# KyungMinJin/OTPose

Hardware: AMD Instinct MI355X
Metric: frames/sec at 384x288, 5-frame window, batch 16; heatmap max-abs delta vs ref (higher is better)
Workload: dtype f32 storage+accumulate / f16x3 split products; 1 GPU; BASELINE configs[1]: batch 16 x 5-frame x 384x288, HRNet-W48 + DCN warp + ConvVideoTransformer, fp32 forward (eval), seeded synthetic weights; clips_per_gpu=16, parallelism=dp1, outputs_finite=True

## Files before the change

### otpose_amd/csrc/convs.hip

```cpp
#include "x3.h"
#include <cstdlib>

namespace {

#ifdef OTP_CONVS_TIMING
__device__ unsigned long long otp_convs_stamps[8192 * 32];
#define SSTAMP(slot)                                                                                  \
    do {                                                                                              \
        if (threadIdx.x == 0 && blockIdx.x < 8192) otp_convs_stamps[blockIdx.x * 32 + (slot)] = __builtin_readcyclecounter(); \
    } while (0)
#else
#define SSTAMP(slot)
#endif

struct SPlan {
    int N, C, H, W, HW, Cout, total;
    int out_ctot, out_coff, act, f32_mode, res_s8;
    float pre, post;
    int NTW, nN, nTiles, nChunks, tpx;
    int NPT;
    int VR, W1, NIW, NV, pl;
    uint32_t mHW, mW, mW1, mVR;
    unsigned* rflag;
};

__global__ __launch_bounds__(256) void s8_pack_kernel(const float* __restrict__ in, otp_u32x4* __restrict__ out, float* __restrict__ c4,
                                                       int N, int C, int HW, int ctot, int coff, unsigned* rflag) {
    const int G8 = C >> 3;
    const size_t items = (size_t)N * G8 * HW;
    bool bad = false;
    for (size_t i = (size_t)blockIdx.x * 256 + threadIdx.x; i < items; i += (size_t)gridDim.x * 256) {
        const int p = (int)(i % HW);
        const size_t r = i / HW;
        const int g = (int)(r % G8), n = (int)(r / G8);
        const float* src = in + ((size_t)n * ctot + coff + 8 * g) * HW + p;
        float f[8];
#pragma unroll
        for (int e = 0; e < 8; ++e) f[e] = src[(size_t)e * HW];
#pragma unroll
        for (int e = 0; e < 8; ++e) bad |= otp_out_of_range(f[e]);
        otp_u32x4 hi, lo;
        otp_x3_split8(f, hi, lo);
        otp_u32x4* dst = out + ((size_t)(n * G8 + g) * 2) * HW + p;
        dst[0] = hi;
        dst[HW] = lo;
        if (c4) {
            otp_f32x4* d4 = reinterpret_cast<otp_f32x4*>(c4) + ((size_t)n * (C >> 2) + 2 * g) * HW + p;
            d4[0] = (otp_f32x4){f[0], f[1], f[2], f[3]};
            d4[HW] = (otp_f32x4){f[4], f[5], f[6], f[7]};
        }
    }
    otp_range_report(rflag, bad, OTP_RANGE_S8PASS);
}

struct S8Up {
    const float* low[3];
    int f[3];
    int n;
};
__global__ __launch_bounds__(256) void s8_upsample_add4_kernel(S8Up U, const float* __restrict__ res, float* out_nchw,
                                                               otp_u32x4* __restrict__ out_s8, float* __restrict__ out_c4, int N, int C,
                                                               int Hh, int Wh, int relu, int res_ctot, int res_coff, int out_ctot,
                                                               int out_coff, int res_s8, unsigned* rflag) {
    const int HW = Hh * Wh, q4 = HW >> 2, G8 = C >> 3, Wh4 = Wh >> 2;
    const size_t items = (size_t)N * G8 * q4;
    bool bad = false;
    for (size_t i = (size_t)blockIdx.x * 256 + threadIdx.x; i < items; i += (size_t)gridDim.x * 256) {
        const int q = (int)(i % q4);
        const size_t r = i / q4;
        const int g = (int)(r % G8), n = (int)(r / G8);
        const int y = q / Wh4, x4 = q - y * Wh4;
        otp_f32x4 v[8];
        if (res_s8) {
            const otp_u32x4* rs = reinterpret_cast<const otp_u32x4*>(res) + ((size_t)(n * G8 + g) * 2) * HW + 4 * q;
#pragma unroll
            for (int k = 0; k < 4; ++k) {
                const otp_u32x4 h = rs[k], l = rs[(size_t)HW + k];
#pragma unroll
                for (int e2 = 0; e2 < 4; ++e2) {
                    const otp_f32x2 a = otp_x3_widen(h[e2]) + otp_x3_widen(l[e2]);
                    v[2 * e2][k] = a.x;
                    v[2 * e2 + 1][k] = a.y;
                }
            }
        }
#pragma unroll
        for (int e = 0; e < 8; ++e) {
            const int c = 8 * g + e;
            otp_f32x4 o = res_s8 ? v[e] : *reinterpret_cast<const otp_f32x4*>(res + ((size_t)n * res_ctot + res_coff + c) * HW + 4 * q);
#pragma unroll
            for (int k = 0; k < 3; ++k) {
                if (k < U.n) {
                    const int f = U.f[k], Wl = Wh / f, Hl = Hh / f;
                    const float* lrow = U.low[k] + (((size_t)n * C + c) * Hl + y / f) * Wl;
                    if (f >= 4) {
                        o = o + lrow[(4 * x4) / f];
                    } else {
                        const float l0 = lrow[2 * x4], l1 = lrow[2 * x4 + 1];
                        o = o + (otp_f32x4){l0, l0, l1, l1};
                    }
                }
            }
#pragma unroll
            for (int j = 0; j < 4; ++j) bad |= otp_out_of_range(o[j]);
            if (relu) {
#pragma unroll
                for (int j = 0; j < 4; ++j) o[j] = fmaxf(o[j], 0.f);
            }
            v[e] = o;
            if (out_nchw) *reinterpret_cast<otp_f32x4*>(out_nchw + ((size_t)n * out_ctot + out_coff + c) * HW + 4 * q) = o;
        }
        otp_u32x4* dst = out_s8 + ((size_t)(n * G8 + g) * 2) * HW + 4 * q;
#pragma unroll
        for (int k = 0; k < 4; ++k) {
            float f[8];
#pragma unroll
            for (int e = 0; e < 8; ++e) f[e] = v[e][k];
            otp_u32x4 hi, lo;
            otp_x3_split8(f, hi, lo);
            dst[k] = hi;
            dst[(size_t)HW + k] = lo;
            if (out_c4) {
                otp_f32x4* d4 = reinterpret_cast<otp_f32x4*>(out_c4) + ((size_t)n * (C >> 2) + 2 * g) * HW + 4 * q + k;
                d4[0] = (otp_f32x4){f[0], f[1], f[2], f[3]};
                d4[HW] = (otp_f32x4){f[4], f[5], f[6], f[7]};
            }
        }
    }
    otp_range_report(rflag, bad, OTP_RANGE_S8PASS);
}

__global__ __launch_bounds__(256) void s8_upsample_add_kernel(S8Up U, const float* __restrict__ res, float* out_nchw,
                                                               otp_u32x4* __restrict__ out_s8, float* __restrict__ out_c4, int N, int C,
                                                               int Hh, int Wh, int relu, int res_ctot, int res_coff, int out_ctot,
                                                               int out_coff, int res_s8, unsigned* rflag) {
    const int HW = Hh * Wh, G8 = C >> 3;
    const size_t items = (size_t)N * G8 * HW;
    bool bad = false;
    for (size_t i = (size_t)blockIdx.x * 256 + threadIdx.x; i < items; i += (size_t)gridDim.x * 256) {
        const int p = (int)(i % HW);
        const size_t r = i / HW;
        const int g = (int)(r % G8), n = (int)(r / G8);
        const int y = p / Wh, x = p - y * Wh;
        int lo_off[3];
#pragma unroll
        for (int k = 0; k < 3; ++k) {
            const int f = k < U.n ? U.f[k] : 1;
            lo_off[k] = (y / f) * (Wh / f) + x / f;
        }
        float f8[8];
        if (res_s8) {
            const otp_u32x4* rs = reinterpret_cast<const otp_u32x4*>(res) + ((size_t)(n * G8 + g) * 2) * HW + p;
            const otp_u32x4 h = rs[0], l = rs[HW];
#pragma unroll
            for (int e2 = 0; e2 < 4; ++e2) {
                const otp_f32x2 a = otp_x3_widen(h[e2]) + otp_x3_widen(l[e2]);
                f8[2 * e2] = a.x;
                f8[2 * e2 + 1] = a.y;
            }
        }
#pragma unroll
        for (int e = 0; e < 8; ++e) {
            const int c = 8 * g + e;
            float o = res_s8 ? f8[e] : res[((size_t)n * res_ctot + res_coff + c) * HW + p];
#pragma unroll
            for (int k = 0; k < 3; ++k) {
                if (k < U.n) {
                    const int f = U.f[k];
                    o = o + U.low[k][((size_t)n * C + c) * (size_t)((Hh / f) * (Wh / f)) + lo_off[k]];
                }
            }
            bad |= otp_out_of_range(o);
            if (relu) o = fmaxf(o, 0.f);
            f8[e] = o;
            if (out_nchw) out_nchw[((size_t)n * out_ctot + out_coff + c) * HW + p] = o;
        }
        otp_u32x4 hi, lo;
        otp_x3_split8(f8, hi, lo);
        otp_u32x4* dst = out_s8 + ((size_t)(n * G8 + g) * 2) * HW + p;
        dst[0] = hi;
        dst[HW] = lo;
        if (out_c4) {
            otp_f32x4* d4 = reinterpret_cast<otp_f32x4*>(out_c4) + ((size_t)n * (C >> 2) + 2 * g) * HW + p;
            d4[0] = (otp_f32x4){f8[0], f8[1], f8[2], f8[3]};
            d4[HW] = (otp_f32x4){f8[4], f8[5], f8[6], f8[7]};
        }
    }
    otp_range_report(rflag, bad, OTP_RANGE_S8PASS);
}

__global__ __launch_bounds__(256) void c4_unpack_kernel(const otp_f32x4* __restrict__ in, float* __restrict__ out, int N, int C, int HW) {
    const size_t items = (size_t)N * (C >> 2) * HW;
    for (size_t i = (size_t)blockIdx.x * 256 + threadIdx.x; i < items; i += (size_t)gridDim.x * 256) {
        const int p = (int)(i % HW);
        const size_t r = i / HW;
        const int c4 = (int)(r % (C >> 2)), n = (int)(r / (C >> 2));
        const otp_f32x4 v = in[i];
#pragma unroll
        for (int e = 0; e < 4; ++e) out[((size_t)n * C + 4 * c4 + e) * HW + p] = v[e];
    }
}

__global__ __launch_bounds__(256) void s8_unpack_kernel(const otp_u32x4* __restrict__ in, float* __restrict__ out, int N, int C, int HW) {
    const int G8 = C >> 3;
    const size_t items = (size_t)N * G8 * HW;
    for (size_t i = (size_t)blockIdx.x * 256 + threadIdx.x; i < items; i += (size_t)gridDim.x * 256) {
        const int p = (int)(i % HW);
        const size_t r = i / HW;
        const int g = (int)(r % G8), n = (int)(r / G8);
        const otp_u32x4 hi = in[((size_t)(n * G8 + g) * 2) * HW + p], lo = in[((size_t)(n * G8 + g) * 2 + 1) * HW + p];
#pragma unroll
        for (int e = 0; e < 8; ++e) {
            const otp_f32x2 fh = otp_x3_widen(hi[e >> 1]), fl = otp_x3_widen(lo[e >> 1]);
            out[((size_t)n * C + 8 * g + e) * HW + p] = fh[e & 1] + fl[e & 1];
        }
    }
}

__global__ void s8_wpack_kernel(const float* __restrict__ w, const float* __restrict__ scale, otp_u32x4* __restrict__ out, int Cout,
                                int Cin, int NTW, int nN, int nChunks) {
    const int total = nN * nChunks * OTP_S8_KS * NTW * 64;
    const int WU = otp_s8_wch(NTW) * 64;
    for (int idx = blockIdx.x * blockDim.x + threadIdx.x; idx < total; idx += gridDim.x * blockDim.x) {
        const int lane = idx & 63;
        int r = idx >> 6;
        const int t = r % NTW; r /= NTW;
        const int s = r % OTP_S8_KS; r /= OTP_S8_KS;
        const int chunk = r % nChunks, cb = r / nChunks;
        const int cout = otp_row2ch(cb * NTW * 16, t, lane & 15, NTW, Cout), kl = lane >> 4;
        const int q = 4 * s + kl, tap = q >> 1, ci0 = chunk * 16 + 8 * (q & 1);
        if (tap > 8) continue;
        float v[8];
#pragma unroll
        for (int j = 0; j < 8; ++j) {
            const int ci = ci0 + j;
            v[j] = (cout < Cout && ci < Cin) ? w[((size_t)cout * Cin + ci) * 9 + tap] * (scale ? scale[cout] : 1.f) : 0.f;
        }
        otp_u32x4 hi, lo;
        otp_x3_split8(v, hi, lo);
        const size_t base = (size_t)(cb * nChunks + chunk) * WU;
        if (s < OTP_S8_KS - 1) {
            const size_t o = base + ((s * NTW + t) * 2) * 64 + lane;
            out[o] = hi;
            out[o + 64] = lo;
        } else {
            const size_t o = base + (OTP_S8_KS - 1) * NTW * 128 + t * 64 + lane;
            out[o] = hi;
            out[o + 32] = lo;
        }
    }
}


template <int NM>
__device__ __forceinline__ void sblock_sched_n(int nr) {
    if (nr == 0) otp_s8_block_sched<NM, 0>();
    else if (nr == 1) otp_s8_block_sched<NM, 1>();
    else if (nr == 2) otp_s8_block_sched<NM, 2>();
    else if (nr == 1 + 2 * 2) otp_s8_block_sched<NM, 1 + 2 * 2>();
    else if (nr == 2 + 2 * 2) otp_s8_block_sched<NM, 2 + 2 * 2>();
    else if (nr == 1 + 2 * 3) otp_s8_block_sched<NM, 1 + 2 * 3>();
    else otp_s8_block_sched<NM, 2 + 2 * 3>();
}

enum { S_F32_NONE = 0, S_F32_C4 = 1, S_F32_NCHW = 2 };

template <int NTW, bool NCHW, int NPT>
__global__ __launch_bounds__(256, NCHW ? 2 : 3) void convs_kernel(const unsigned char* __restrict__ xs, const otp_u32x4* __restrict__ wpk,
                                                        const float* __restrict__ shift, const float* res, float* outf,
                                                        otp_u32x4* outs, const SPlan P) {
    constexpr int BM = 64 * NPT;
    constexpr int WCH = otp_s8_wch(NTW);
    constexpr int WBYTES = WCH * 1024;
    constexpr int NBLK = OTP_S8_KS * NPT;
    constexpr int NM = 3 * NTW;
    extern __shared__ __attribute__((aligned(16))) unsigned char smem[];
    const int PL = P.pl;
    unsigned char* win = smem;
    unsigned char* wl = smem + 4 * PL;
    const int tid = threadIdx.x, lane = tid & 63;
    const int wave = __builtin_amdgcn_readfirstlane(tid >> 6);
    const int i16 = lane & 15, kl = lane >> 4;
    const bool upper = kl >= 2;

    const int xcd = (int)blockIdx.x & 7, jb = (int)blockIdx.x >> 3;
    const int tl = jb / P.nN, cb = jb - tl * P.nN;
    const int tile = xcd * P.tpx + tl;
    if (tile >= P.nTiles) return;
    SSTAMP(0);
#ifdef OTP_CONVS_TIMING
    if (threadIdx.x == 0 && blockIdx.x < 8192) otp_convs_stamps[blockIdx.x * 32 + 30] = __builtin_amdgcn_s_memrealtime();
#endif
    const int P0 = tile * BM;
    const int n0 = P0 / P.HW, p0 = P0 - n0 * P.HW;
    const int y0 = (int)otp_magic_div((uint32_t)p0, P.mW);
    const int x0 = p0 - y0 * P.W;
    const int Vf = n0 * P.VR + y0;
    const int imgB = P.C * P.HW * 4;
    const int co_blk = cb * NTW * 16;
    const int C4o = P.Cout >> 2;

    int voff[2];
    bool vlive[2];
#pragma unroll
    for (int j = 0; j < 2; ++j) {
        vlive[j] = 64 * (wave + 4 * j) + lane < P.NV;
        const int v = 64 * (wave + 4 * j) + lane + x0;
        const int r = (int)otp_magic_div((uint32_t)v, P.mW1), cp = v - otp_mul24(r, P.W1);
        const int V = Vf + r;
        const int n = (int)otp_magic_div((uint32_t)V, P.mVR), yy = V - otp_mul24(n, P.VR);
        const bool ok = cp >= 1 && yy >= 1 && n < P.N;
        voff[j] = ok ? (n - n0) * imgB + (otp_mul24(yy - 1, P.W) + cp - 1) * 16 : OTP_OOB;
    }
    const size_t left = (size_t)(P.N - n0) * imgB;
    const otp_rsrc rin = make_rsrc32(xs + (size_t)n0 * imgB, left > 0x7fffff00ull ? 0x7fffff00u : (unsigned)left);
    const otp_rsrc rw = make_rsrc32(wpk, (unsigned)((size_t)P.nN * P.nChunks * WBYTES));
    const int woff = lane * 16;

    auto stage = [&](int c) __attribute__((always_inline)) {
#pragma unroll
        for (int pl = 0; pl < 4; ++pl) {
            const int so = (((2 * c + (pl >> 1)) * 2 + (pl & 1)) * P.HW) * 16;
#pragma unroll
            for (int j = 0; j < 2; ++j) {
                const int k = wave + 4 * j;
                if (k < P.NIW && vlive[j])
                    __builtin_amdgcn_raw_ptr_buffer_load_lds(rin, (__attribute__((address_space(3))) void*)(win + pl * PL + k * 1024),
                                                             16, voff[j], so, 0, 0);
            }
        }
        const int wb = (cb * P.nChunks + c) * WBYTES;
#pragma unroll
        for (int j = 0; j < (WCH + 3) / 4; ++j) {
            const int k = wave + 4 * j;
            if (k < WCH)
                __builtin_amdgcn_raw_ptr_buffer_load_lds(rw, (__attribute__((address_space(3))) void*)(wl + k * 1024), 16, woff,
                                                         wb + k * 1024, 0, 0);
        }
    };
    stage(0);
    SSTAMP(1);

    const size_t obytes = (size_t)P.N * P.Cout * P.HW * 4;
    const otp_rsrc rres = make_rsrc32(res ? res : reinterpret_cast<const float*>(xs), res ? (unsigned)obytes : 0u);
    const otp_rsrc rs8 = make_rsrc32(outs, outs ? (unsigned)obytes : 0u);
    const otp_rsrc rof = make_rsrc32(outf, !outf ? 0u : (P.f32_mode == S_F32_C4 ? (unsigned)obytes
                                                                               : (unsigned)((size_t)P.N * P.out_ctot * P.HW * 4)));
    const otp_rsrc rsh = make_rsrc32(shift ? shift : reinterpret_cast<const float*>(xs), shift ? (unsigned)(P.Cout * 4) : 0u);
    int pb[NPT], toff[OTP_S8_KS], offN[NCHW ? NPT : 1], offS[NPT], ch0[NTW];
    otp_f32x4 acc[NTW][NPT];
    {
#pragma unroll
        for (int s = 0; s < OTP_S8_KS; ++s) {
            const int q = 4 * s + kl;
            int tap = q >> 1;
            if (tap > 8) tap = 8;
            const int dy = tap / 3, dx = tap - dy * 3;
            toff[s] = (dy * P.W1 + dx - x0) * 16 + (q & 1) * (2 * PL);
        }
        if (upper) toff[OTP_S8_KS - 1] += PL;
        otp_f32x4 sh[NTW];
#pragma unroll
        for (int t = 0; t < NTW; ++t) {
            ch0[t] = otp_row2ch(co_blk, t, 4 * kl, NTW, P.Cout);
            sh[t] = __builtin_bit_cast(otp_f32x4, __builtin_amdgcn_raw_buffer_load_b128(rsh, co_blk + 16 * t < P.Cout ? ch0[t] * 4 : OTP_OOB, 0, 0));
        }
#pragma unroll
        for (int p = 0; p < NPT; ++p) {
            int m = (wave * NPT + p) * 16 + i16;
            const bool pv = P0 + m < P.total;
            if (!pv) m = P.total - 1 - P0;
            const int q = p0 + m;
            const int dn = (int)otp_magic_div((uint32_t)q, P.mHW), pi = q - otp_mul24(dn, P.HW);
            const int y = (int)otp_magic_div((uint32_t)pi, P.mW), x = pi - otp_mul24(y, P.W);
            pb[p] = (otp_mul24(otp_mul24(n0 + dn, P.VR) + y - Vf, P.W1) + x) * 16;
            const int img = n0 + dn;
            const int c4o = (otp_mul24(otp_mul24(img, C4o), P.HW) + pi) * 16;
            if (NCHW) offN[NCHW ? p : 0] = pv ? (otp_mul24(otp_mul24(img, P.out_ctot) + P.out_coff, P.HW) + pi) * 4 : OTP_OOB;
            offS[p] = pv ? c4o : OTP_OOB;
            if (!P.res_s8) {
#pragma unroll
                for (int t = 0; t < NTW; ++t) {
                    const bool tv = co_blk + 16 * t < P.Cout;
                    acc[t][p] = __builtin_bit_cast(otp_f32x4, __builtin_amdgcn_raw_buffer_load_b128(
                        rres, (pv && tv) ? c4o + otp_mul24(ch0[t] >> 2, P.HW) * 16 : OTP_OOB, 0, 0));
                }
            }
        }
        if (P.res_s8) {
#pragma unroll
            for (int t = 1; t < NTW; t += 2)
#pragma unroll
                for (int p = 0; p < NPT; ++p) acc[t][p] = otp_f32x4{0.f, 0.f, 0.f, 0.f};
#pragma unroll
            for (int t = 0; t < NTW; t += 2) {
                const bool tav = co_blk + 16 * t < P.Cout;
                const int so = otp_mul24(ch0[t] >> 3, P.HW) * 32;
                if (otp_tile_paired(co_blk, t, NTW, P.Cout)) {
#pragma unroll
                    for (int p = 0; p < NPT; ++p) {
                        const int o = (tav && offS[p] != OTP_OOB) ? offS[p] + so : OTP_OOB;
                        const otp_u32x4 h = __builtin_bit_cast(otp_u32x4, __builtin_amdgcn_raw_buffer_load_b128(rres, o, 0, 0));
                        const otp_u32x4 l = __builtin_bit_cast(otp_u32x4, __builtin_amdgcn_raw_buffer_load_b128(rres, o, P.HW * 16, 0));
                        const otp_f32x2 a0 = otp_x3_widen(h[0]) + otp_x3_widen(l[0]), a1 = otp_x3_widen(h[1]) + otp_x3_widen(l[1]);
                        const otp_f32x2 a2 = otp_x3_widen(h[2]) + otp_x3_widen(l[2]), a3 = otp_x3_widen(h[3]) + otp_x3_widen(l[3]);
                        acc[t][p] = otp_f32x4{a0.x, a0.y, a1.x, a1.y};
                        acc[t + 1 < NTW ? t + 1 : t][p] = otp_f32x4{a2.x, a2.y, a3.x, a3.y};
                    }
                } else {
                    const int half = (ch0[t] >> 2) & 1;
#pragma unroll
                    for (int p = 0; p < NPT; ++p) {
                        const int o = (tav && offS[p] != OTP_OOB) ? offS[p] + so + 8 * half : OTP_OOB;
                        const otp_u32x2 h = __builtin_bit_cast(otp_u32x2, __builtin_amdgcn_raw_buffer_load_b64(rres, o, 0, 0));
                        const otp_u32x2 l = __builtin_bit_cast(otp_u32x2, __builtin_amdgcn_raw_buffer_load_b64(rres, o, P.HW * 16, 0));
                        const otp_f32x2 a0 = otp_x3_widen(h[0]) + otp_x3_widen(l[0]), a1 = otp_x3_widen(h[1]) + otp_x3_widen(l[1]);
                        acc[t][p] = otp_f32x4{a0.x, a0.y, a1.x, a1.y};
                    }
                }
            }
        }
#pragma unroll
        for (int t = 0; t < NTW; ++t) {
            const otp_f32x4 shp = sh[t] * P.pre;
#pragma unroll
            for (int p = 0; p < NPT; ++p) acc[t][p] = acc[t][p] * P.pre + shp;
        }
    }

    auto mfma_phase = [&]() __attribute__((always_inline)) {
        otp_x3x8 ah[2][NTW], al[2][NTW], bh[3], bl[3];
        auto load_a = [&](int buf, int s) __attribute__((always_inline)) {
#pragma unroll
            for (int t = 0; t < NTW; ++t) {
                if (s < OTP_S8_KS - 1) {
                    const unsigned char* a = wl + ((s * NTW + t) * 2) * 1024 + lane * 16;
                    ah[buf][t] = *reinterpret_cast<const otp_x3x8*>(a);
                    al[buf][t] = *reinterpret_cast<const otp_x3x8*>(a + 1024);
                } else {
                    const unsigned char* a = wl + (OTP_S8_KS - 1) * NTW * 2048 + t * 1024;
                    const otp_x3x8 h = *reinterpret_cast<const otp_x3x8*>(a + (lane & 31) * 16);
                    const otp_x3x8 z = __builtin_bit_cast(otp_x3x8, (otp_u32x4){0u, 0u, 0u, 0u});
                    al[buf][t] = *reinterpret_cast<const otp_x3x8*>(a + (lane ^ 32) * 16);
                    ah[buf][t] = upper ? z : h;
                }
            }
        };
        auto load_b = [&](int buf, int blk) __attribute__((always_inline)) {
            const unsigned char* b = win + (pb[blk % NPT] + toff[blk / NPT]);
            bh[buf] = *reinterpret_cast<const otp_x3x8*>(b);
            if (blk / NPT < OTP_S8_KS - 1) bl[buf] = *reinterpret_cast<const otp_x3x8*>(b + PL);
        };
        load_a(0, 0);
        load_b(0, 0);
        load_b(1, 1);
#pragma unroll
        for (int blk = 0; blk < NBLK; ++blk) {
            const int s = blk / NPT, p = blk % NPT, cur = blk % 3, sa = s & 1;
            const bool nb = blk + 2 < NBLK, na = p == NPT - 2 && s + 1 < OTP_S8_KS;
            if (nb) load_b((blk + 2) % 3, blk + 2);
            if (na) load_a(sa ^ 1, s + 1);
            const int nr = (nb ? ((blk + 2) / NPT < OTP_S8_KS - 1 ? 2 : 1) : 0) + (na ? 2 * NTW : 0);
            if (s < OTP_S8_KS - 1) {
#pragma unroll
                for (int t = 0; t < NTW; ++t) {
                    acc[t][p] = OTP_X3_MFMA(al[sa][t], bh[cur], acc[t][p], 0, 0, 0);
                    acc[t][p] = OTP_X3_MFMA(ah[sa][t], bl[cur], acc[t][p], 0, 0, 0);
                    acc[t][p] = OTP_X3_MFMA(ah[sa][t], bh[cur], acc[t][p], 0, 0, 0);
                }
                sblock_sched_n<NM>(nr);
            } else {
#pragma unroll
                for (int t = 0; t < NTW; ++t) {
                    acc[t][p] = OTP_X3_MFMA(al[sa][t], bh[cur], acc[t][p], 0, 0, 0);
                    acc[t][p] = OTP_X3_MFMA(ah[sa][t], bh[cur], acc[t][p], 0, 0, 0);
                }
                sblock_sched_n<2 * NTW>(nr);
            }
            __builtin_amdgcn_sched_barrier(0);
        }
    };

    SSTAMP(2);
    for (int c = 0; c < P.nChunks; ++c) {
        asm volatile("s_waitcnt vmcnt(0)" ::: "memory");
        if (c < 3) SSTAMP(3 + 4 * c);
        __syncthreads();
        if (c < 3) SSTAMP(4 + 4 * c);
        mfma_phase();
        if (c < 3) SSTAMP(5 + 4 * c);
        if (c + 1 < P.nChunks) {
            __syncthreads();
            stage(c + 1);
        }
        if (c < 3) SSTAMP(6 + 4 * c);
    }
    SSTAMP(16);

    if (P.post != 1.f) {
#pragma unroll
        for (int t = 0; t < NTW; ++t)
#pragma unroll
            for (int p = 0; p < NPT; ++p) acc[t][p] = acc[t][p] * P.post;
    }
    {
        bool bad = false;
#pragma unroll
        for (int t = 0; t < NTW; ++t)
#pragma unroll
            for (int p = 0; p < NPT; ++p)
#pragma unroll
                for (int r = 0; r < 4; ++r) bad |= otp_out_of_range(acc[t][p][r]);
        otp_range_report(P.rflag, bad, OTP_RANGE_CONVS);
    }
    if (P.act == OTP_ACT_RELU) {
#pragma unroll
        for (int t = 0; t < NTW; ++t)
#pragma unroll
            for (int p = 0; p < NPT; ++p)
#pragma unroll
                for (int r = 0; r < 4; ++r) acc[t][p][r] = otp_relu(acc[t][p][r]);
    }
    otp_u32x4 rec[(NTW + 1) / 2][NPT][2];
    if (outs) {
#pragma unroll
        for (int t = 0; t < NTW; t += 2) {
            const bool paired = otp_tile_paired(co_blk, t, NTW, P.Cout);
            const int t1 = t + 1 < NTW ? t + 1 : t;
#pragma unroll
            for (int p = 0; p < NPT; ++p) {
                const float f[8] = {acc[t][p][0], acc[t][p][1], acc[t][p][2], acc[t][p][3],
                                    paired ? acc[t1][p][0] : 0.f, paired ? acc[t1][p][1] : 0.f,
                                    paired ? acc[t1][p][2] : 0.f, paired ? acc[t1][p][3] : 0.f};
                otp_x3_split8(f, rec[t >> 1][p][0], rec[t >> 1][p][1]);
            }
        }
    }
    SSTAMP(17);
    if (!NCHW && P.f32_mode == S_F32_C4) {
#pragma unroll
        for (int t = 0; t < NTW; ++t)
#pragma unroll
            for (int p = 0; p < NPT; ++p)
                __builtin_amdgcn_raw_buffer_store_b128(__builtin_bit_cast(otp_u32x4, acc[t][p]), rof,
                                                       (co_blk + 16 * t < P.Cout && offS[p] != OTP_OOB) ? offS[p] + otp_mul24(ch0[t] >> 2, P.HW) * 16 : OTP_OOB,
                                                       0, 0);
    } else if (NCHW) {
        constexpr int RS = BM + 4;
        float* tl = reinterpret_cast<float*>(smem);
        __syncthreads();
#pragma unroll
        for (int t = 0; t < NTW; ++t)
#pragma unroll
            for (int p = 0; p < NPT; ++p)
#pragma unroll
                for (int r = 0; r < 4; ++r)
                    tl[(ch0[t] - co_blk + r) * RS + (wave * NPT + p) * 16 + i16] = acc[t][p][r];
        __syncthreads();
        constexpr int G = BM / 4, CPI = 256 / G;
        const int g = tid % G, c0 = tid / G;
        const bool gv = P0 + 4 * g < P.total;
        const int q = gv ? p0 + 4 * g : p0;
        const int qn = (int)otp_magic_div((uint32_t)q, P.mHW), qi = q - otp_mul24(qn, P.HW);
        const int ob = gv ? (otp_mul24(otp_mul24(n0 + qn, P.out_ctot) + P.out_coff + co_blk, P.HW) + qi) * 4 : OTP_OOB;
#pragma unroll
        for (int k = 0; k < NTW * 16 / CPI; ++k) {
            const int ch = c0 + CPI * k;
            const otp_u32x4 v = *reinterpret_cast<const otp_u32x4*>(tl + ch * RS + 4 * g);
            __builtin_amdgcn_raw_buffer_store_b128(v, rof, (ob != OTP_OOB && co_blk + ch < P.Cout) ? ob + otp_mul24(ch, P.HW) * 4 : OTP_OOB, 0, 0);
        }
    }
    if (outs) {
#pragma unroll
        for (int t = 0; t < NTW; t += 2) {
            const bool tav = co_blk + 16 * t < P.Cout;
            const int so = otp_mul24(ch0[t] >> 3, P.HW) * 32;
            if (otp_tile_paired(co_blk, t, NTW, P.Cout)) {
#pragma unroll
                for (int p = 0; p < NPT; ++p) {
                    const int o = offS[p] != OTP_OOB ? offS[p] + so : OTP_OOB;
                    __builtin_amdgcn_raw_buffer_store_b128(rec[t >> 1][p][0], rs8, o, 0, 0);
                    __builtin_amdgcn_raw_buffer_store_b128(rec[t >> 1][p][1], rs8, o, P.HW * 16, 0);
                }
            } else {
                const int half = (ch0[t] >> 2) & 1;
#pragma unroll
                for (int p = 0; p < NPT; ++p) {
                    const int o = (tav && offS[p] != OTP_OOB) ? offS[p] + so + 8 * half : OTP_OOB;
                    __builtin_amdgcn_raw_buffer_store_b64((otp_u32x2){rec[t >> 1][p][0][0], rec[t >> 1][p][0][1]}, rs8, o, 0, 0);
                    __builtin_amdgcn_raw_buffer_store_b64((otp_u32x2){rec[t >> 1][p][1][0], rec[t >> 1][p][1][1]}, rs8, o, P.HW * 16, 0);
                }
            }
        }
    }
    SSTAMP(19);
#ifdef OTP_CONVS_TIMING
    if (threadIdx.x == 0 && blockIdx.x < 8192) otp_convs_stamps[blockIdx.x * 32 + 31] = __builtin_amdgcn_s_memrealtime();
#endif
}

int force_npt() {
    static const int v = [] {
        const char* e = getenv("OTPOSE_S8_NPT");
        return e ? atoi(e) : 0;
    }();
    return v;
}

int s8_ntw(int Cout) {
    const int c16 = (Cout + 15) / 16;
    return (c16 % 3 == 0) ? 3 : (c16 % 2 == 0 || c16 <= 2 ? 2 : 3);
}

bool convs_plan(const otp_conv_desc& d, SPlan& P) {
    if (d.kh != 3 || d.kw != 3 || d.stride != 1 || d.pad != 1 || d.dil != 1) return false;
    if (d.res_up > 1 || d.frame_split > 0 || d.in2_ctot > 0 || d.act == OTP_ACT_GELU) return false;
    if (d.Cin % 16 || d.Cout % 16 || ((d.H * d.W) & 3) || d.Ho != d.H || d.Wo != d.W) return false;
    P.N = d.N; P.C = d.Cin; P.H = d.H; P.W = d.W; P.HW = d.H * d.W; P.Cout = d.Cout; P.total = d.N * P.HW;
    P.out_ctot = d.out_ctot; P.out_coff = d.out_coff; P.act = d.act; P.f32_mode = S_F32_NONE;
    P.post = d.out_scale > 0.f ? d.out_scale : 1.f;
    P.pre = 1.f / P.post;
    P.res_s8 = d.res_layout == 1;
    P.NTW = s8_ntw(d.Cout);
    P.nN = ((d.Cout + 15) / 16 + P.NTW - 1) / P.NTW;
    P.NPT = 4;
    if ((long)((P.total + 255) / 256) * P.nN < 3 * 256 && force_npt() != 4) P.NPT = 2;
    if (force_npt() == 2) P.NPT = 2;
    const int bm = 64 * P.NPT;
    P.nTiles = (P.total + bm - 1) / bm;
    P.nChunks = d.Cin / 16;
    P.tpx = (P.nTiles + 7) / 8;
    P.VR = d.H + 1;
    P.W1 = d.W + 1;
    int NV = 0;
    for (int t = 0; t < P.nTiles; ++t) {
        const int a = t * bm, b = (a + bm < P.total ? a + bm : P.total) - 1;
        const int na = a / P.HW, ya = (a % P.HW) / d.W, xa = (a % P.HW) % d.W;
        const int nb = b / P.HW, yb = (b % P.HW) / d.W, xb = (b % P.HW) % d.W;
        const int rows = (nb * P.VR + yb + 1) - (na * P.VR + ya);
        const int v = (rows + 1) * P.W1 + xb - xa + 3;
        if (v > NV) NV = v;
    }
    if (NV > 512) return false;
    P.NV = NV;
    P.pl = NV * 16;
    P.NIW = (NV + 63) / 64;
    P.mHW = otp_magic(P.HW); P.mW = otp_magic(d.W); P.mW1 = otp_magic(P.W1); P.mVR = otp_magic(P.VR);
    if ((long)(P.HW + bm) * P.HW >= (1l << 32) || (long)P.HW * d.W >= (1l << 32)) return false;
    if ((long)(d.N + 1) * P.VR * P.VR >= (1l << 32)) return false;
    {
        const long span = (long)(bm) / P.HW + 2;
        if (span * d.Cin * P.HW * 4 >= (1l << 31)) return false;
    }
    if (P.HW < 32) return false;
    if (P.HW >= (1 << 24) || (long)(d.N + 8) * P.VR >= (1l << 24) || (long)(d.N + 8) * (d.Cout / 4 + d.out_ctot) + d.out_coff >= (1l << 24)) return false;
    if ((size_t)P.nN * P.nChunks * otp_s8_wch(P.NTW) * 1024 >= (1ull << 31)) return false;
    return true;
}

template <int NTW, bool NCHW, int NPT>
int convs_launch(const void* xs, const void* wpk, const float* shift, const float* res, float* outf, void* outs, const SPlan& P,
                 hipStream_t st) {
    auto kern = convs_kernel<NTW, NCHW, NPT>;
    size_t need = (size_t)4 * P.pl + otp_s8_wch(NTW) * 1024;
    if (NCHW && need < (size_t)NTW * 16 * (64 * NPT + 4) * 4) need = (size_t)NTW * 16 * (64 * NPT + 4) * 4;
    OTP_ALLOW_BIG_LDS(kern, need);
    hipLaunchKernelGGL(kern, dim3(8 * P.tpx * P.nN), dim3(256), need, st, static_cast<const unsigned char*>(xs),
                       static_cast<const otp_u32x4*>(wpk), shift, res, outf, static_cast<otp_u32x4*>(outs), P);
    return otp_launch_status();
}

}

#ifdef OTP_CONVS_TIMING
extern "C" int otp_convs_read_stamps(void* host_out, size_t bytes) {
    return hipMemcpyFromSymbol(host_out, HIP_SYMBOL(otp_convs_stamps), bytes) == hipSuccess ? OTP_OK : OTP_ERR_LAUNCH;
}
#endif

extern "C" size_t otp_s8_bytes(int N, int C, int H, int W) {
    if (N <= 0 || C <= 0 || H <= 0 || W <= 0 || C % 8) return 0;
    return (size_t)N * C * H * W * 4;
}

extern "C" int otp_s8_pack(const void* in, void* out, void* out_c4, int N, int C, int H, int W, int in_ctot, int in_coff,
                           void* stream) {
    if (!in || !out || N <= 0 || C <= 0 || H <= 0 || W <= 0 || in_ctot < in_coff + C || in_coff < 0) return OTP_ERR_BAD_ARG;
    if (C % 8 || ((H * W) & 3) ||
        ((reinterpret_cast<uintptr_t>(in) | reinterpret_cast<uintptr_t>(out) | reinterpret_cast<uintptr_t>(out_c4)) & 15))
        return OTP_ERR_UNSUPPORTED;
    const size_t items = (size_t)N * (C / 8) * (H * W);
    const int grid = (int)((items + 255) / 256 > 16384 ? 16384 : (items + 255) / 256);
    hipLaunchKernelGGL(s8_pack_kernel, dim3(grid), dim3(256), 0, static_cast<hipStream_t>(stream), static_cast<const float*>(in),
                       static_cast<otp_u32x4*>(out), static_cast<float*>(out_c4), N, C, H * W, in_ctot, in_coff, otp_range_word());
    return otp_launch_status();
}

extern "C" int otp_s8_upsample_add(const void* const* lows, const int* factors, int nlow, const void* res, void* out_nchw,
                                   void* out_s8, void* out_c4, int N, int C, int Hh, int Wh, int relu, int res_ctot, int res_coff,
                                   int out_ctot, int out_coff, void* stream) {
    return otp_s8_upsample_add_ex(lows, factors, nlow, res, 0, out_nchw, out_s8, out_c4, N, C, Hh, Wh, relu, res_ctot, res_coff,
                                  out_ctot, out_coff, stream);
}

extern "C" int otp_s8_upsample_add_ex(const void* const* lows, const int* factors, int nlow, const void* res, int res_layout,
                                      void* out_nchw, void* out_s8, void* out_c4, int N, int C, int Hh, int Wh, int relu,
                                      int res_ctot, int res_coff, int out_ctot, int out_coff, void* stream) {
    if (!lows || !factors || !res || !out_s8 || nlow < 1 || nlow > 3 || N <= 0 || C <= 0 || Hh <= 0 || Wh <= 0)
        return OTP_ERR_BAD_ARG;
    if (res_layout != 0 && res_layout != 1) return OTP_ERR_BAD_ARG;
    const int res_s8 = res_layout;
    if (Wh % 4 || C % 8 || (!res_s8 && res_ctot < res_coff + C) || (out_nchw && out_ctot < out_coff + C)) return OTP_ERR_UNSUPPORTED;
    S8Up U{};
    U.n = nlow;
    for (int k = 0; k < nlow; ++k) {
        const int f = factors[k];
        if (!lows[k]) return OTP_ERR_BAD_ARG;
        if (f < 2 || (f & (f - 1)) || Hh % f || Wh % f) return OTP_ERR_UNSUPPORTED;
        U.low[k] = static_cast<const float*>(lows[k]);
        U.f[k] = f;
    }
    if ((reinterpret_cast<uintptr_t>(res) | reinterpret_cast<uintptr_t>(out_nchw) | reinterpret_cast<uintptr_t>(out_s8) |
         reinterpret_cast<uintptr_t>(out_c4)) & 15)
        return OTP_ERR_UNSUPPORTED;
    if (nlow >= 3) {
        const size_t items4 = (size_t)N * (C / 8) * (Hh * Wh / 4);
        const int grid4 = (int)((items4 + 255) / 256 > 8192 ? 8192 : (items4 + 255) / 256);
        hipLaunchKernelGGL(s8_upsample_add4_kernel, dim3(grid4), dim3(256), 0, static_cast<hipStream_t>(stream), U,
                           static_cast<const float*>(res), static_cast<float*>(out_nchw), static_cast<otp_u32x4*>(out_s8),
                           static_cast<float*>(out_c4), N, C, Hh, Wh, relu, res_ctot, res_coff, out_ctot, out_coff, res_s8, otp_range_word());
        return otp_launch_status();
    }
    const size_t items = (size_t)N * (C / 8) * (Hh * Wh);
    const int grid = (int)((items + 255) / 256 > 16384 ? 16384 : (items + 255) / 256);
    hipLaunchKernelGGL(s8_upsample_add_kernel, dim3(grid), dim3(256), 0, static_cast<hipStream_t>(stream), U,
                       static_cast<const float*>(res), static_cast<float*>(out_nchw), static_cast<otp_u32x4*>(out_s8),
                       static_cast<float*>(out_c4), N, C, Hh, Wh, relu, res_ctot, res_coff, out_ctot, out_coff, res_s8, otp_range_word());
    return otp_launch_status();
}

extern "C" int otp_s8_unpack(const void* in, void* out, int N, int C, int H, int W, void* stream) {
    if (!in || !out || N <= 0 || C <= 0 || H <= 0 || W <= 0) return OTP_ERR_BAD_ARG;
    if (C % 8) return OTP_ERR_UNSUPPORTED;
    const size_t items = (size_t)N * (C / 8) * H * W;
    const int grid = (int)((items + 255) / 256 > 8192 ? 8192 : (items + 255) / 256);
    hipLaunchKernelGGL(s8_unpack_kernel, dim3(grid), dim3(256), 0, static_cast<hipStream_t>(stream), static_cast<const otp_u32x4*>(in),
                       static_cast<float*>(out), N, C, H * W);
    return otp_launch_status();
}

extern "C" int otp_c4_unpack(const void* in, void* out, int N, int C, int H, int W, void* stream) {
    if (!in || !out || N <= 0 || C <= 0 || H <= 0 || W <= 0) return OTP_ERR_BAD_ARG;
    if (C % 4) return OTP_ERR_UNSUPPORTED;
    const size_t items = (size_t)N * (C / 4) * H * W;
    const int grid = (int)((items + 255) / 256 > 8192 ? 8192 : (items + 255) / 256);
    hipLaunchKernelGGL(c4_unpack_kernel, dim3(grid), dim3(256), 0, static_cast<hipStream_t>(stream), static_cast<const otp_f32x4*>(in),
                       static_cast<float*>(out), N, C, H * W);
    return otp_launch_status();
}

extern "C" int otp_conv3x3_s8_supported(const otp_conv_desc* desc) {
    if (!desc) return 0;
    SPlan P{};
    return convs_plan(*desc, P) ? 1 : 0;
}

extern "C" size_t otp_conv3x3_s8_weight_bytes(int Cout, int Cin) {
    if (Cout <= 0 || Cin <= 0 || Cin % 16) return 0;
    const int NTW = s8_ntw(Cout), nN = ((Cout + 15) / 16 + NTW - 1) / NTW;
    return (size_t)nN * (Cin / 16) * otp_s8_wch(NTW) * 1024;
}

extern "C" int otp_conv3x3_s8_pack_weight(const void* weight, const void* scale, void* wpacked, int Cout, int Cin, void* stream) {
    if (!weight || !wpacked || Cout <= 0 || Cin <= 0) return OTP_ERR_BAD_ARG;
    if (!otp_conv3x3_s8_weight_bytes(Cout, Cin)) return OTP_ERR_UNSUPPORTED;
    const int NTW = s8_ntw(Cout), nN = ((Cout + 15) / 16 + NTW - 1) / NTW, nChunks = Cin / 16;
    const int total = nN * nChunks * OTP_S8_KS * NTW * 64;
    hipLaunchKernelGGL(s8_wpack_kernel, dim3(otp_ceil_div(total, 256) > 2048 ? 2048 : otp_ceil_div(total, 256)), dim3(256), 0,
                       static_cast<hipStream_t>(stream), static_cast<const float*>(weight), static_cast<const float*>(scale),
                       static_cast<otp_u32x4*>(wpacked), Cout, Cin, NTW, nN, nChunks);
    return otp_launch_status();
}

extern "C" int otp_conv3x3_s8(const void* in_s8, const void* wpacked, const void* shift, const void* res_c4, void* out_f32,
                              int out_f32_layout, void* out_s8, const otp_conv_desc* desc, void* stream) {
    if (!in_s8 || !wpacked || !desc || (!out_f32 && !out_s8)) return OTP_ERR_BAD_ARG;
    const otp_conv_desc& d = *desc;
    if (d.N <= 0 || d.Cin <= 0 || d.Cout <= 0 || d.H <= 0 || d.W <= 0) return OTP_ERR_BAD_ARG;
    if (out_f32 && out_f32_layout != OTP_S8_F32_C4 && out_f32_layout != OTP_S8_F32_NCHW) return OTP_ERR_BAD_ARG;
    if (out_f32 && out_f32_layout == OTP_S8_F32_NCHW && d.out_ctot < d.out_coff + d.Cout) return OTP_ERR_BAD_ARG;
    if ((reinterpret_cast<uintptr_t>(in_s8) | reinterpret_cast<uintptr_t>(wpacked) | reinterpret_cast<uintptr_t>(out_f32) |
         reinterpret_cast<uintptr_t>(out_s8) | reinterpret_cast<uintptr_t>(res_c4) | reinterpret_cast<uintptr_t>(shift)) & 15)
        return OTP_ERR_UNSUPPORTED;
    SPlan P{};
    if (!convs_plan(d, P)) return OTP_ERR_UNSUPPORTED;
    P.rflag = otp_range_word();
    P.f32_mode = out_f32 ? (out_f32_layout == OTP_S8_F32_C4 ? S_F32_C4 : S_F32_NCHW) : S_F32_NONE;
    auto st = static_cast<hipStream_t>(stream);
    auto fs = static_cast<const float*>(shift);
    auto fr = static_cast<const float*>(res_c4);
    auto fo = static_cast<float*>(out_f32);
#define OTP_CONVS_GO(NTW_, NCHW_, NPT_) return convs_launch<NTW_, NCHW_, NPT_>(in_s8, wpacked, fs, fr, fo, out_s8, P, st)
    const bool nchw = P.f32_mode == S_F32_NCHW;
    if (P.NPT == 2) {
        if (P.NTW == 2) { if (nchw) OTP_CONVS_GO(2, true, 2); OTP_CONVS_GO(2, false, 2); }
        if (nchw) OTP_CONVS_GO(3, true, 2);
        OTP_CONVS_GO(3, false, 2);
    }
    if (P.NTW == 2) { if (nchw) OTP_CONVS_GO(2, true, 4); OTP_CONVS_GO(2, false, 4); }
    if (nchw) OTP_CONVS_GO(3, true, 4);
    OTP_CONVS_GO(3, false, 4);
#undef OTP_CONVS_GO
}
```

Before: 3219 frames/s.

## Replace HRNet fuse/upsample and pack kernels with 3D-grid templated buffer-load kernels

The s8 pack kernel now uses a 3D grid (pixel tile, channel group, batch), which removes per-element 64-bit div/mod index math. The upsample-add fuse pass gets a new templated kernel, specialised on the number of low-res inputs, residual layout and output options. Each thread handles a vertical pixel pair so low-res values are shared across the two rows, and loads and stores go through raw buffer descriptors with magic-number division. This aims to cut address arithmetic and redundant low-res loads, but adds 24 template instantiations and relies on power-of-two factors and 32-bit offset limits.

```diff
diff --git a/otpose_amd/csrc/convs.hip b/otpose_amd/csrc/convs.hip
--- a/otpose_amd/csrc/convs.hip
+++ b/otpose_amd/csrc/convs.hip
@@ -27,27 +27,27 @@
 __global__ __launch_bounds__(256) void s8_pack_kernel(const float* __restrict__ in, otp_u32x4* __restrict__ out, float* __restrict__ c4,
                                                        int N, int C, int HW, int ctot, int coff, unsigned* rflag) {
     const int G8 = C >> 3;
-    const size_t items = (size_t)N * G8 * HW;
+    const size_t p0 = (size_t)blockIdx.x * 256;
+    if (p0 + threadIdx.x >= (size_t)HW) return;
     bool bad = false;
-    for (size_t i = (size_t)blockIdx.x * 256 + threadIdx.x; i < items; i += (size_t)gridDim.x * 256) {
-        const int p = (int)(i % HW);
-        const size_t r = i / HW;
-        const int g = (int)(r % G8), n = (int)(r / G8);
-        const float* src = in + ((size_t)n * ctot + coff + 8 * g) * HW + p;
+    for (int n = blockIdx.z; n < N; n += gridDim.z)
+    for (int g = blockIdx.y; g < G8; g += gridDim.y) {
+        const int ng = n * G8 + g;
+        const float* src = in + ((size_t)n * ctot + coff + 8 * g) * HW + p0;
         float f[8];
 #pragma unroll
-        for (int e = 0; e < 8; ++e) f[e] = src[(size_t)e * HW];
+        for (int e = 0; e < 8; ++e) f[e] = (src + (size_t)e * HW)[threadIdx.x];
 #pragma unroll
         for (int e = 0; e < 8; ++e) bad |= otp_out_of_range(f[e]);
         otp_u32x4 hi, lo;
         otp_x3_split8(f, hi, lo);
-        otp_u32x4* dst = out + ((size_t)(n * G8 + g) * 2) * HW + p;
-        dst[0] = hi;
-        dst[HW] = lo;
+        otp_u32x4* dst = out + (size_t)ng * 2 * HW + p0;
+        dst[threadIdx.x] = hi;
+        (dst + HW)[threadIdx.x] = lo;
         if (c4) {
-            otp_f32x4* d4 = reinterpret_cast<otp_f32x4*>(c4) + ((size_t)n * (C >> 2) + 2 * g) * HW + p;
-            d4[0] = (otp_f32x4){f[0], f[1], f[2], f[3]};
-            d4[HW] = (otp_f32x4){f[4], f[5], f[6], f[7]};
+            otp_f32x4* d4 = reinterpret_cast<otp_f32x4*>(c4) + ((size_t)n * (C >> 2) + 2 * g) * HW + p0;
+            d4[threadIdx.x] = (otp_f32x4){f[0], f[1], f[2], f[3]};
+            (d4 + HW)[threadIdx.x] = (otp_f32x4){f[4], f[5], f[6], f[7]};
         }
     }
     otp_range_report(rflag, bad, OTP_RANGE_S8PASS);
@@ -58,76 +58,109 @@
     int f[3];
     int n;
 };
-__global__ __launch_bounds__(256) void s8_upsample_add4_kernel(S8Up U, const float* __restrict__ res, float* out_nchw,
-                                                               otp_u32x4* __restrict__ out_s8, float* __restrict__ out_c4, int N, int C,
-                                                               int Hh, int Wh, int relu, int res_ctot, int res_coff, int out_ctot,
-                                                               int out_coff, int res_s8, unsigned* rflag) {
-    const int HW = Hh * Wh, q4 = HW >> 2, G8 = C >> 3, Wh4 = Wh >> 2;
-    const size_t items = (size_t)N * G8 * q4;
+struct S8Fuse {
+    const float* low[3];
+    int sh[3];
+    int N, C, Hh, Wh, relu, res_ctot, res_coff, out_ctot, out_coff;
+    uint32_t mW;
+    unsigned* rflag;
+};
+
+template <int NLOW, bool RES_S8, bool NCHW_OUT, bool C4_OUT>
+__global__ __launch_bounds__(256) void s8_fuse_pass_kernel(S8Fuse U, const void* __restrict__ res, float* __restrict__ out_nchw,
+                                                           otp_u32x4* __restrict__ out_s8, float* __restrict__ out_c4) {
+    const uint32_t Wh = (uint32_t)U.Wh, HW = (uint32_t)(U.Hh * U.Wh);
+    const uint32_t t = blockIdx.x * 256u + threadIdx.x;
+    if (t >= (HW >> 1)) return;
+    const uint32_t r = otp_magic_div(t, U.mW), x = t - r * Wh;
+    const int pa = (int)(t + r * Wh);
+    int lo_off[NLOW];
+#pragma unroll
+    for (int k = 0; k < NLOW; ++k) lo_off[k] = (int)((((r >> (U.sh[k] - 1)) * (Wh >> U.sh[k])) + (x >> U.sh[k])) * 4u);
+    const int G8 = U.C >> 3;
+    const int rowB = (int)(Wh * 16u), partB = (int)(HW * 16u);
     bool bad = false;
-    for (size_t i = (size_t)blockIdx.x * 256 + threadIdx.x; i < items; i += (size_t)gridDim.x * 256) {
-        const int q = (int)(i % q4);
-        const size_t r = i / q4;
-        const int g = (int)(r % G8), n = (int)(r / G8);
-        const int y = q / Wh4, x4 = q - y * Wh4;
-        otp_f32x4 v[8];
-        if (res_s8) {
-            const otp_u32x4* rs = reinterpret_cast<const otp_u32x4*>(res) + ((size_t)(n * G8 + g) * 2) * HW + 4 * q;
-#pragma unroll
-            for (int k = 0; k < 4; ++k) {
-                const otp_u32x4 h = rs[k], l = rs[(size_t)HW + k];
+    for (int n = blockIdx.z; n < U.N; n += gridDim.z)
+    for (int g = blockIdx.y; g < G8; g += gridDim.y) {
+        const size_t ng = (size_t)n * G8 + g;
+        float v[2][8], l[NLOW][8];
+        otp_u32x4 rh[2], rl[2];
+        if constexpr (RES_S8) {
+            const otp_rsrc rr = make_rsrc32(static_cast<const char*>(res) + ng * 2 * HW * 16, 2u * HW * 16u);
+#pragma unroll
+            for (int j = 0; j < 2; ++j) {
+                rh[j] = __builtin_bit_cast(otp_u32x4, __builtin_amdgcn_raw_buffer_load_b128(rr, pa * 16, j * rowB, 0));
+                rl[j] = __builtin_bit_cast(otp_u32x4, __builtin_amdgcn_raw_buffer_load_b128(rr, pa * 16, partB + j * rowB, 0));
+            }
+        } else {
+            const otp_rsrc rr = make_rsrc32(static_cast<const float*>(res) + ((size_t)n * U.res_ctot + U.res_coff + 8 * g) * HW, 8u * HW * 4u);
+#pragma unroll
+            for (int e = 0; e < 8; ++e) {
+                v[0][e] = bload(rr, pa * 4, (int)(e * HW * 4u));
+                v[1][e] = bload(rr, pa * 4, (int)((e * HW + Wh) * 4u));
+            }
+        }
+#pragma unroll
+        for (int k = 0; k < NLOW; ++k) {
+            const uint32_t plane = HW >> (2 * U.sh[k]);
+            const otp_rsrc rk = make_rsrc32(U.low[k] + ((size_t)n * U.C + 8 * g) * plane, 8u * plane * 4u);
+#pragma unroll
+            for (int e = 0; e < 8; ++e) l[k][e] = bload(rk, lo_off[k], (int)(e * plane * 4u));
+        }
+        if constexpr (RES_S8) {
+#pragma unroll
+            for (int j = 0; j < 2; ++j)
 #pragma unroll
                 for (int e2 = 0; e2 < 4; ++e2) {
-                    const otp_f32x2 a = otp_x3_widen(h[e2]) + otp_x3_widen(l[e2]);
-                    v[2 * e2][k] = a.x;
-                    v[2 * e2 + 1][k] = a.y;
+                    const otp_f32x2 a = otp_x3_widen(rh[j][e2]) + otp_x3_widen(rl[j][e2]);
+                    v[j][2 * e2] = a.x;
+                    v[j][2 * e2 + 1] = a.y;
                 }
-            }
         }
 #pragma unroll
         for (int e = 0; e < 8; ++e) {
-            const int c = 8 * g + e;
-            otp_f32x4 o = res_s8 ? v[e] : *reinterpret_cast<const otp_f32x4*>(res + ((size_t)n * res_ctot + res_coff + c) * HW + 4 * q);
-#pragma unroll
-            for (int k = 0; k < 3; ++k) {
-                if (k < U.n) {
-                    const int f = U.f[k], Wl = Wh / f, Hl = Hh / f;
-                    const float* lrow = U.low[k] + (((size_t)n * C + c) * Hl + y / f) * Wl;
-                    if (f >= 4) {
-                        o = o + lrow[(4 * x4) / f];
-                    } else {
-                        const float l0 = lrow[2 * x4], l1 = lrow[2 * x4 + 1];
-                        o = o + (otp_f32x4){l0, l0, l1, l1};
-                    }
-                }
-            }
-#pragma unroll
-            for (int j = 0; j < 4; ++j) bad |= otp_out_of_range(o[j]);
-            if (relu) {
-#pragma unroll
-                for (int j = 0; j < 4; ++j) o[j] = fmaxf(o[j], 0.f);
-            }
-            v[e] = o;
-            if (out_nchw) *reinterpret_cast<otp_f32x4*>(out_nchw + ((size_t)n * out_ctot + out_coff + c) * HW + 4 * q) = o;
-        }
-        otp_u32x4* dst = out_s8 + ((size_t)(n * G8 + g) * 2) * HW + 4 * q;
-#pragma unroll
-        for (int k = 0; k < 4; ++k) {
-            float f[8];
-#pragma unroll
-            for (int e = 0; e < 8; ++e) f[e] = v[e][k];
+#pragma unroll
+            for (int j = 0; j < 2; ++j) {
+                float o = v[j][e];
+#pragma unroll
+                for (int k = 0; k < NLOW; ++k) o = o + l[k][e];
+                bad |= otp_out_of_range(o);
+                v[j][e] = o;
+            }
+        }
+        if (U.relu) {
+#pragma unroll
+            for (int e = 0; e < 8; ++e) {
+                v[0][e] = otp_relu(v[0][e]);
+                v[1][e] = otp_relu(v[1][e]);
+            }
+        }
+        if constexpr (NCHW_OUT) {
+            const otp_rsrc ro = make_rsrc32(out_nchw + ((size_t)n * U.out_ctot + U.out_coff + 8 * g) * HW, 8u * HW * 4u);
+#pragma unroll
+            for (int e = 0; e < 8; ++e) {
+                bstore(v[0][e], ro, pa * 4, (int)(e * HW * 4u));
+                bstore(v[1][e], ro, pa * 4, (int)((e * HW + Wh) * 4u));
+            }
+        }
+        const otp_rsrc rs = make_rsrc32(reinterpret_cast<char*>(out_s8) + ng * 2 * HW * 16, 2u * HW * 16u);
+        otp_rsrc rc;
+        if constexpr (C4_OUT) rc = make_rsrc32(reinterpret_cast<char*>(out_c4) + ((size_t)n * (U.C >> 2) + 2 * g) * HW * 16, 2u * HW * 16u);
+#pragma unroll
+        for (int j = 0; j < 2; ++j) {
             otp_u32x4 hi, lo;
-            otp_x3_split8(f, hi, lo);
-            dst[k] = hi;
-            dst[(size_t)HW + k] = lo;
-            if (out_c4) {
-                otp_f32x4* d4 = reinterpret_cast<otp_f32x4*>(out_c4) + ((size_t)n * (C >> 2) + 2 * g) * HW + 4 * q + k;
-                d4[0] = (otp_f32x4){f[0], f[1], f[2], f[3]};
-                d4[HW] = (otp_f32x4){f[4], f[5], f[6], f[7]};
-            }
-        }
-    }
-    otp_range_report(rflag, bad, OTP_RANGE_S8PASS);
+            otp_x3_split8(v[j], hi, lo);
+            __builtin_amdgcn_raw_buffer_store_b128(hi, rs, pa * 16, j * rowB, 0);
+            __builtin_amdgcn_raw_buffer_store_b128(lo, rs, pa * 16, partB + j * rowB, 0);
+            if constexpr (C4_OUT) {
+                __builtin_amdgcn_raw_buffer_store_b128(__builtin_bit_cast(otp_u32x4, (otp_f32x4){v[j][0], v[j][1], v[j][2], v[j][3]}), rc,
+                                                       pa * 16, j * rowB, 0);
+                __builtin_amdgcn_raw_buffer_store_b128(__builtin_bit_cast(otp_u32x4, (otp_f32x4){v[j][4], v[j][5], v[j][6], v[j][7]}), rc,
+                                                       pa * 16, partB + j * rowB, 0);
+            }
+        }
+    }
+    otp_range_report(U.rflag, bad, OTP_RANGE_S8PASS);
 }
 
 __global__ __launch_bounds__(256) void s8_upsample_add_kernel(S8Up U, const float* __restrict__ res, float* out_nchw,
@@ -689,9 +722,9 @@
     if (C % 8 || ((H * W) & 3) ||
         ((reinterpret_cast<uintptr_t>(in) | reinterpret_cast<uintptr_t>(out) | reinterpret_cast<uintptr_t>(out_c4)) & 15))
         return OTP_ERR_UNSUPPORTED;
-    const size_t items = (size_t)N * (C / 8) * (H * W);
-    const int grid = (int)((items + 255) / 256 > 16384 ? 16384 : (items + 255) / 256);
-    hipLaunchKernelGGL(s8_pack_kernel, dim3(grid), dim3(256), 0, static_cast<hipStream_t>(stream), static_cast<const float*>(in),
+    const int G8 = C / 8;
+    const dim3 grid((unsigned)((H * W + 255) / 256), (unsigned)(G8 > 65535 ? 65535 : G8), (unsigned)(N > 65535 ? 65535 : N));
+    hipLaunchKernelGGL(s8_pack_kernel, grid, dim3(256), 0, static_cast<hipStream_t>(stream), static_cast<const float*>(in),
                        static_cast<otp_u32x4*>(out), static_cast<float*>(out_c4), N, C, H * W, in_ctot, in_coff, otp_range_word());
     return otp_launch_status();
 }
@@ -712,30 +745,50 @@
     const int res_s8 = res_layout;
     if (Wh % 4 || C % 8 || (!res_s8 && res_ctot < res_coff + C) || (out_nchw && out_ctot < out_coff + C)) return OTP_ERR_UNSUPPORTED;
     S8Up U{};
+    S8Fuse F{};
     U.n = nlow;
     for (int k = 0; k < nlow; ++k) {
         const int f = factors[k];
         if (!lows[k]) return OTP_ERR_BAD_ARG;
         if (f < 2 || (f & (f - 1)) || Hh % f || Wh % f) return OTP_ERR_UNSUPPORTED;
-        U.low[k] = static_cast<const float*>(lows[k]);
+        U.low[k] = F.low[k] = static_cast<const float*>(lows[k]);
         U.f[k] = f;
+        F.sh[k] = __builtin_ctz((unsigned)f);
     }
     if ((reinterpret_cast<uintptr_t>(res) | reinterpret_cast<uintptr_t>(out_nchw) | reinterpret_cast<uintptr_t>(out_s8) |
          reinterpret_cast<uintptr_t>(out_c4)) & 15)
         return OTP_ERR_UNSUPPORTED;
-    if (nlow >= 3) {
-        const size_t items4 = (size_t)N * (C / 8) * (Hh * Wh / 4);
-        const int grid4 = (int)((items4 + 255) / 256 > 8192 ? 8192 : (items4 + 255) / 256);
-        hipLaunchKernelGGL(s8_upsample_add4_kernel, dim3(grid4), dim3(256), 0, static_cast<hipStream_t>(stream), U,
-                           static_cast<const float*>(res), static_cast<float*>(out_nchw), static_cast<otp_u32x4*>(out_s8),
-                           static_cast<float*>(out_c4), N, C, Hh, Wh, relu, res_ctot, res_coff, out_ctot, out_coff, res_s8, otp_range_word());
+    const hipStream_t st = static_cast<hipStream_t>(stream);
+    const size_t HW = (size_t)Hh * Wh;
+    if ((HW / 2) * (size_t)Wh < (1ull << 32) && HW <= (1u << 26)) {
+        F.N = N; F.C = C; F.Hh = Hh; F.Wh = Wh; F.relu = relu;
+        F.res_ctot = res_ctot; F.res_coff = res_coff; F.out_ctot = out_ctot; F.out_coff = out_coff;
+        F.mW = otp_magic((uint32_t)Wh);
+        F.rflag = otp_range_word();
+        const int G8 = C / 8;
+        const dim3 grid((unsigned)((HW / 2 + 255) / 256), (unsigned)(G8 > 65535 ? 65535 : G8), (unsigned)(N > 65535 ? 65535 : N));
+        const int pick = ((nlow - 1) * 2 + res_s8) * 4 + (out_nchw ? 2 : 0) + (out_c4 ? 1 : 0);
+        switch (pick) {
+#define OTP_FUSE_CASE(I, NL, RS, NC, C4)                                                                                          \
+    case I:                                                                                                                        \
+        hipLaunchKernelGGL((s8_fuse_pass_kernel<NL, RS, NC, C4>), grid, dim3(256), 0, st, F, res, static_cast<float*>(out_nchw), \
+                           static_cast<otp_u32x4*>(out_s8), static_cast<float*>(out_c4));                                          \
+        break;
+#define OTP_FUSE_CASES4(I, NL, RS)                                                                                                \
+    OTP_FUSE_CASE(I, NL, RS, false, false) OTP_FUSE_CASE(I + 1, NL, RS, false, true) OTP_FUSE_CASE(I + 2, NL, RS, true, false)     \
+    OTP_FUSE_CASE(I + 3, NL, RS, true, true)
+            OTP_FUSE_CASES4(0, 1, false) OTP_FUSE_CASES4(4, 1, true) OTP_FUSE_CASES4(8, 2, false) OTP_FUSE_CASES4(12, 2, true)
+            OTP_FUSE_CASES4(16, 3, false) OTP_FUSE_CASES4(20, 3, true)
+#undef OTP_FUSE_CASES4
+#undef OTP_FUSE_CASE
+        }
         return otp_launch_status();
     }
-    const size_t items = (size_t)N * (C / 8) * (Hh * Wh);
+    const size_t items = (size_t)N * (C / 8) * HW;
     const int grid = (int)((items + 255) / 256 > 16384 ? 16384 : (items + 255) / 256);
-    hipLaunchKernelGGL(s8_upsample_add_kernel, dim3(grid), dim3(256), 0, static_cast<hipStream_t>(stream), U,
-                       static_cast<const float*>(res), static_cast<float*>(out_nchw), static_cast<otp_u32x4*>(out_s8),
-                       static_cast<float*>(out_c4), N, C, Hh, Wh, relu, res_ctot, res_coff, out_ctot, out_coff, res_s8, otp_range_word());
+    hipLaunchKernelGGL(s8_upsample_add_kernel, dim3(grid), dim3(256), 0, st, U, static_cast<const float*>(res),
+                       static_cast<float*>(out_nchw), static_cast<otp_u32x4*>(out_s8), static_cast<float*>(out_c4), N, C, Hh, Wh, relu,
+                       res_ctot, res_coff, out_ctot, out_coff, res_s8, otp_range_word());
     return otp_launch_status();
 }
 
```

Result: faster. 3285 frames/s (median of 6 runs) (+2.0%).
